# madmann91/bvh

Measured on AMD Instinct MI355X. Metric: Mrays/s closest-hit (1M-tri scene), higher is better.
Workload: dtype f32; 1 GPU; soup_1m: 1,000,000-triangle random soup (M3), worst-case incoherent; robust traversal, DefaultBuilder with thread pool (mini-trees) Quality::High built on the GPU (the reference's default configuration is thread pool + High); rays reordered for coherence inside the timed pass (library default for this tree size); tris=1000000, nodes=1866439, ray_batches=4, parallelism=single GPU, launched_by=single process

## Files before the change

bvh_amd/__init__.py:

```python
from .api import (BinnedSahBuilder, MiniTreeBuilder, SplitHeuristic, Bvh, Config, DefaultBuilder, Quality, RayFlags, SweepSahBuilder, ThreadPool, prepare_trace,
                  HITD, HITF, INVALID, NODED, NODEF, NODE2D, NODE2F, closest_points, hits_to_numpy, intersect, precompute_tris, sphere_bounds,
                  tri_bounds, gather, radius_count, radius_search, offsets_from_counts, ray_hit_count, ray_hits, ray_hits_nearest, RAY_NEAREST_MAX_K, knn, KNN_MAX_K, overlap_count, overlap_search, self_overlaps, instance_prepare, intersect_instanced, std_sort_ids, radix_sort_pairs, reinsertion_stats, last_optimize_profile, pinhole_rays, shade_eyelight)
from ._lib import BvhAmdError
```

bvh_amd/_lib.py:

```python
from __future__ import annotations

import ctypes as C
import os

HERE = os.path.dirname(os.path.abspath(__file__))
LIB_PATH = os.environ.get("BVH_AMD_LIB") or os.path.join(HERE, "lib", "libbvh_amd.so")

_lib = None


class BvhAmdError(RuntimeError):
    pass


class BuildConfig(C.Structure):
    _fields_ = [("quality", C.c_int), ("min_leaf_size", C.c_size_t), ("max_leaf_size", C.c_size_t),
                ("parallel_threshold", C.c_size_t)]


class Counters(C.Structure):
    _fields_ = [("node_pairs", C.c_ulonglong), ("prim_tests", C.c_ulonglong), ("leaves", C.c_ulonglong)]


class MiniTreeConfig(C.Structure):
# ... 58 lines not shown
    "bvh_thread_pool_create": (_P, [_Z]),
    "bvh_thread_pool_destroy": (None, [_P]),
    "bvh_amd_gather": (_I, [_P, _P, _Z, _Z, _P, _P]),
    "bvh_amd_pinhole_rays3f": (_I, [_P, _P, _P, _Z, _Z, _P, _P]),
    "bvh_amd_pinhole_rays3d": (_I, [_P, _P, _P, _Z, _Z, _P, _P]),
    "bvh_amd_shade_eyelight3f": (_I, [_P, _P, _P, _Z, _P, _P]),
    "bvh_amd_shade_eyelight3d": (_I, [_P, _P, _P, _Z, _P, _P]),
    "bvh_amd_device_alloc": (_P, [_Z]),
    "bvh_amd_device_free": (None, [_P]),
    "bvh_amd_copy_to_device": (_I, [_P, _P, _Z]),
    "bvh_amd_copy_to_host": (_I, [_P, _P, _Z]),
    "bvh_amd_synchronize": (_I, [_P]),
    "bvh_amd_std_sort_ids3f": (_I, [_P, _Z, _P, _P]),
    "bvh_amd_std_sort_ids3d": (_I, [_P, _Z, _P, _P]),
    "bvh_amd_radix_sort_pairs_u32": (_I, [_P, _P, _Z, _I, _P]),
    "bvh_amd_offsets_from_counts": (_I, [_P, _Z, _P, _P]),
}
_SIGS_T = {
    "bvh{S}_build": (_P, [_P, _P, _P, _Z, _P]),
    "bvh{S}_build_device": (_P, [_P, _P, _Z, _P, _I, _P]),
    "bvh{S}_build_sah": (_P, [_P, _P, _P, _Z, _P, _P]),
    "bvh{S}_build_device_sah": (_P, [_P, _P, _Z, _P, _I, _P, _P]),
    "bvh{S}_build_device_binned": (_P, [_P, _P, _Z, _P, _P, _Z, _P]),
    "bvh{S}_build_minitree_device": (_P, [_P, _P, _Z, _P, _P]),
    "bvh{S}_from_nodes": (_P, [_P, _Z, _P, _Z]),
    "bvh{S}_extract": (_P, [_P, _Z]),
    "bvh{S}_destroy": (None, [_P]),
    "bvh{S}_optimize": (None, [_P, _P]),
    "bvh{S}_optimize_config": (_I, [_P, _P]),
    "bvh{S}_refit": (None, [_P]),
# ... 136 lines not shown
```

bvh_amd/api.py:

```python
from __future__ import annotations

import ctypes as C
import enum
from dataclasses import dataclass, field

import numpy as np

from . import _lib

INVALID = 0xFFFFFFFF
HITF = np.dtype([("prim", "<u4"), ("t", "<f4"), ("u", "<f4"), ("v", "<f4")])
HITD = np.dtype([("prim", "<u4"), ("pad", "<u4"), ("t", "<f8"), ("u", "<f8"), ("v", "<f8")])
NODEF = np.dtype([("bounds", "<f4", (6,)), ("index", "<u4")])
NODED = np.dtype([("bounds", "<f8", (6,)), ("index", "<u8")])
NODE2F = np.dtype([("bounds", "<f4", (4,)), ("index", "<u4")])
NODE2D = np.dtype([("bounds", "<f8", (4,)), ("index", "<u8")])
_NODE_DTYPES = {"3f": NODEF, "3d": NODED, "2f": NODE2F, "2d": NODE2D}


class Quality(enum.IntEnum):
    Low = 0
    Medium = 1
    High = 2

# ... 758 lines not shown
def std_sort_ids(keys):
    torch = _torch()
    k = _dev(keys).reshape(-1)
    s = _suffix(k.dtype)
    out = torch.empty(k.shape[0], dtype=torch.int32, device=k.device)
    _lib.check(getattr(_lib.load(), f"bvh_amd_std_sort_ids{s}")(k.data_ptr(), k.shape[0], out.data_ptr(), _stream()), "std_sort_ids")
    return out


def radix_sort_pairs(keys_u32, vals_u32, bits=32):
    torch = _torch()
    k = _dev(keys_u32).to(torch.int32).clone()
    v = _dev(vals_u32).to(torch.int32).clone()
    _lib.check(_lib.load().bvh_amd_radix_sort_pairs_u32(k.data_ptr(), v.data_ptr(), k.shape[0], bits, _stream()), "radix_sort_pairs")
    return k, v
```

bvh_amd/csrc/capi.hip:

```cpp
#include "common.h"

#include <cstring>
#include <memory>
#include <type_traits>

namespace bvh_amd {

template <typename T> int reinsertion_optimize_device(HostNode<T>* d_nodes, size_t node_count, hipStream_t stream, int dim);
template <typename T>
int reinsertion_optimize_config_device(HostNode<T>* d_nodes, size_t node_count, hipStream_t stream, int dim, double batch_size_ratio, size_t iterations);
void reinsertion_stats(unsigned out[2]);
void last_optimize_profile(bvh_amd_optimize_profile* out);
template <typename T>
int build_minitree_explicit(BvhImpl<T>& out, const T* d_bboxes, const T* d_centers, size_t n, const bvh_build_config& cfg, bool prune, T ratio,
                            bool optimize, uint32_t log2_grid, hipStream_t stream);
template <typename T>
int extract_device(BvhImpl<T>& out, const HostNode<T>* d_nodes, size_t node_count, const uint32_t* d_ids, size_t root_id, hipStream_t stream);
template <typename T> int refit_device(HostNode<T>* d_nodes, size_t node_count, hipStream_t stream);
template <typename T> int reachable_node_count(const HostNode<T>* d_nodes, size_t node_count, hipStream_t stream, size_t* out);
template <typename T> int relayout_on_device(BvhImpl<T>& b, const HostNode<T>* d_nodes, hipStream_t stream);

namespace {
thread_local std::string g_error;
}
// ... 805 lines not shown
int bvh_amd_std_sort_ids3f(const float* d_keys, size_t n, uint32_t* d_ids_out, void* stream) {
    return std_sort_ids<float>(d_ids_out, d_keys, static_cast<uint32_t>(n), 1, 0, 1, static_cast<hipStream_t>(stream));
}
int bvh_amd_std_sort_ids3d(const double* d_keys, size_t n, uint32_t* d_ids_out, void* stream) {
    return std_sort_ids<double>(d_ids_out, d_keys, static_cast<uint32_t>(n), 1, 0, 1, static_cast<hipStream_t>(stream));
}
int bvh_amd_radix_sort_pairs_u32(uint32_t* d_keys, uint32_t* d_vals, size_t n, int bits, void* stream) {
    DeviceTemps<uint32_t> tmp;
    auto& [kt, vt] = tmp;
    BVH_HIP_TRY(hipMalloc(&kt, std::max<size_t>(n, 1) * 4), BVH_AMD_ERR_HIP);
    hipError_t e = hipMalloc(&vt, std::max<size_t>(n, 1) * 4);
    return e == hipSuccess ? radix_sort_pairs<uint32_t>(d_keys, d_vals, kt, vt, static_cast<uint32_t>(n), 1, bits, static_cast<hipStream_t>(stream))
                           : fail(BVH_AMD_ERR_HIP, hipGetErrorString(e));
}

int bvh_amd_pinhole_rays3f(const float eye[3], const float dir[3], const float up[3], size_t w, size_t h, bvh_ray3f* d_rays, void* stream) {
    return launch_pinhole_rays<float>(eye, dir, up, w, h, reinterpret_cast<float*>(d_rays), static_cast<hipStream_t>(stream));
}
int bvh_amd_pinhole_rays3d(const double eye[3], const double dir[3], const double up[3], size_t w, size_t h, bvh_ray3d* d_rays, void* stream) {
    return launch_pinhole_rays<double>(eye, dir, up, w, h, reinterpret_cast<double*>(d_rays), static_cast<hipStream_t>(stream));
}
int bvh_amd_shade_eyelight3f(const float* d_tris12, const bvh_ray3f* d_rays, const bvh_hit3f* d_hits, size_t n, uint8_t* d_rgb, void* stream) {
    return launch_shade_eyelight<float>(d_tris12, reinterpret_cast<const float*>(d_rays), d_hits, n, d_rgb, static_cast<hipStream_t>(stream));
}
int bvh_amd_shade_eyelight3d(const double* d_tris12, const bvh_ray3d* d_rays, const bvh_hit3d* d_hits, size_t n, uint8_t* d_rgb, void* stream) {
    return launch_shade_eyelight<double>(d_tris12, reinterpret_cast<const double*>(d_rays), d_hits, n, d_rgb, static_cast<hipStream_t>(stream));
}

int bvh_amd_gather(const void* d_in, const uint32_t* d_perm, size_t n, size_t stride, void* d_out, void* stream) {
    return launch_gather(d_in, d_perm, n, stride, d_out, static_cast<hipStream_t>(stream));
// ... 4 lines not shown
```

bvh_amd/csrc/common.h:

```cpp
#pragma once

#include <hip/hip_runtime.h>

#include <cstddef>
#include <cstdint>
#include <cstring>
#include <string>
#include <atomic>
#include <mutex>
#include <vector>

#include "../../include/bvh_amd.h"

namespace bvh_amd {

constexpr unsigned kCountBits = 4;
constexpr uint32_t kCountMask = 15u;
constexpr int kWave = 64;

template <typename T> struct IndexOf;
template <> struct IndexOf<float>  { using Type = uint32_t; };
template <> struct IndexOf<double> { using Type = uint64_t; };

template <typename T>
// ... 216 lines not shown
template <typename T> int launch_sphere_bounds(const T* d_sph4, size_t n, T* d_bb, T* d_cc, hipStream_t s);
int launch_gather(const void* d_in, const uint32_t* d_perm, size_t n, size_t stride, void* d_out, hipStream_t s);
template <typename T> int launch_circle_bounds(const T* d_circles3, size_t n, T* d_bb4, T* d_cc2, hipStream_t s);
template <typename T> int launch_widen_inputs(const T* d_bb4, const T* d_cc2, size_t n, T* d_bb6, T* d_cc3, hipStream_t s);

template <typename T> int launch_pinhole_rays(const T eye[3], const T dir[3], const T up[3], size_t width, size_t height, T* d_rays, hipStream_t s);
template <typename T>
int launch_shade_eyelight(const T* d_tris12, const T* d_rays, const typename HitOf<T>::Type* d_hits, size_t n, uint8_t* d_rgb, hipStream_t s);

template <typename K>
int radix_sort_pairs(K* keys, uint32_t* vals, K* keys_tmp, uint32_t* vals_tmp, uint32_t n, uint32_t batch, int bits, hipStream_t stream,
                     uint32_t* hist_buf = nullptr, bool iota_vals = false, bool keys_wanted = true, uint32_t** vals_result = nullptr,
                     bool first_hist_done = false);
constexpr int kRadixTileU32 = 8192;
size_t radix_sort_hist_words(uint32_t n, uint32_t batch);
template <typename T>
int std_sort_ids(uint32_t* d_ids, const T* d_keys, uint32_t n, uint32_t batch, uint32_t astride, uint32_t istride, hipStream_t stream);

int exclusive_scan_u32(const uint32_t* in, uint32_t* out, uint32_t n, uint32_t* total_host, hipStream_t stream);

template <typename T>
int build_on_device(BvhImpl<T>& out, const T* d_bboxes, const T* d_centers, size_t n, const bvh_build_config& cfg,
                    bvh_amd_builder builder, hipStream_t stream);

enum { LEAF_TRIANGLE = 0, LEAF_SPHERE = 1 };

enum { REFIT_BOXES3 = 0, REFIT_BOXES2 = 1, REFIT_TRIS = 2 };
template <typename T>
int refit_prims_device(HostNode<T>* d_nodes, PairNode<T>* d_pairs, size_t node_count, int src_kind, const T* d_src, size_t n_src,
                       const uint32_t* d_prim_ids, size_t prim_count, hipStream_t stream);
// ... 5 lines not shown
```

bvh_amd/csrc/query_order.h:

```cpp
#pragma once

#include <algorithm>
#include <string>

namespace bvh_amd {

namespace {

enum QueryKind : int { kQueryPoints = 0, kQueryBoxes = 1, kQueryRays = 2 };

template <typename T>
__global__ void __launch_bounds__(1024) closest_keys_kernel(const T* queries, uint32_t n, T lx, T ly, T lz, T sx, T sy, T sz, uint32_t cells,
                                                            uint32_t* keys, uint32_t* hist, uint32_t tiles) {
    __shared__ uint32_t h[256];
    if (threadIdx.x < 256) h[threadIdx.x] = 0;
    __syncthreads();
    const uint32_t base = blockIdx.x * uint32_t(kRadixTileU32);
#pragma unroll
    for (int s0 = 0; s0 < kRadixTileU32 / 1024; ++s0) {
        const uint32_t i = base + uint32_t(s0) * 1024u + threadIdx.x;
        if (i < n) {
            T q[4];
            load_prim4(queries + 4ull * i, q);
            const T r[8] = { q[0], q[1], q[2], T(0), T(0), T(0), T(0), q[3] };
// ... 45 lines not shown
            load_ray(rays + 8ull * i, r);
            const int hilbert_bits = 31 - __clz(cells);
            const uint32_t key = ray_key<T>(r, lx, ly, lz, sx, sy, sz, cells, hilbert_bits, 0, T(0));
            keys[i] = key;
            atomicAdd(&h[key & 0xFFu], 1u);
        }
    }
    __syncthreads();
    if (threadIdx.x < 256) hist[size_t{threadIdx.x} * tiles + blockIdx.x] = h[threadIdx.x];
}

template <typename T, int Kind = kQueryPoints>
int query_order(const BvhImpl<T>& b, const T* d_queries, size_t n, int cell_bits, const char* who, hipStream_t stream, void** sort_mem,
                ScratchTag* sort_tag, const uint32_t** order_out) {
    const uint32_t n32 = static_cast<uint32_t>(n);
    const size_t words = 4 * n + radix_sort_hist_words(n32, 1);
    const hipError_t e = scratch_alloc(sort_mem, words * sizeof(uint32_t), sort_tag);
    if (e != hipSuccess) { *sort_mem = nullptr; return fail(BVH_AMD_ERR_HIP, std::string(who) + ": no scratch for the query sort: " + hipGetErrorString(e)); }
    uint32_t *keys = static_cast<uint32_t*>(*sort_mem), *vals = keys + n, *kt = vals + n, *vt = kt + n, *hist = vt + n;
    const uint32_t cells = 1u << cell_bits;
    T lo[3], sc[3];
    if (const int rc0 = b.wait_refit()) return rc0;
    for (int k = 0; k < 3; ++k) {
        const T ext = b.root_bounds[2 * k + 1] - b.root_bounds[2 * k];
        lo[k] = b.root_bounds[2 * k];
        sc[k] = ext > T(0) ? T(cells) / ext : T(0);
    }
    const uint32_t tiles = (n32 + kRadixTileU32 - 1) / kRadixTileU32;
    if constexpr (Kind == kQueryRays)
        hipLaunchKernelGGL(ray_query_keys_kernel<T>, dim3(tiles), dim3(1024), 0, stream, d_queries, n32, lo[0], lo[1], lo[2], sc[0], sc[1], sc[2], cells,
                           keys, hist, tiles);
    else if constexpr (Kind == kQueryBoxes)
        hipLaunchKernelGGL(box_keys_kernel<T>, dim3(tiles), dim3(1024), 0, stream, d_queries, n32, lo[0], lo[1], lo[2], sc[0], sc[1], sc[2], cells,
                           keys, hist, tiles);
    else
        hipLaunchKernelGGL(closest_keys_kernel<T>, dim3(tiles), dim3(1024), 0, stream, d_queries, n32, lo[0], lo[1], lo[2], sc[0], sc[1], sc[2], cells,
                           keys, hist, tiles);
    BVH_HIP_TRY(hipGetLastError(), BVH_AMD_ERR_HIP);
    uint32_t* order = nullptr;
    const int rc = radix_sort_pairs<uint32_t>(keys, vals, kt, vt, n32, 1, 3 * cell_bits + 3, stream, hist, true, false, &order,
                                              true);
    if (rc) return rc;
    *order_out = order;
    return BVH_AMD_OK;
}

}

}
```

bvh_amd/csrc/sort_emul.hip:

```cpp

#include "build_common.h"

namespace bvh_amd {

using namespace bld;

namespace {

template <typename K> struct RadixShape {
    static constexpr int kTile = sizeof(K) == 2 || sizeof(K) == 4 ? 8192 : 4096;
    static constexpr int kThreads = kTile / 16;
    static constexpr int kWaves = kThreads / 64;
};
constexpr int kRadixMinTile = 4096;

template <typename K>
__global__ void __launch_bounds__(RadixShape<K>::kThreads) k_radix_hist(const K* keys, uint32_t n, uint32_t blocks_per_array, int shift,
                                                                       uint32_t* hist) {
    constexpr int kTile = RadixShape<K>::kTile, kThreads = RadixShape<K>::kThreads;
    __shared__ uint32_t h[256];
    const uint32_t arr = blockIdx.x / blocks_per_array, blk = blockIdx.x % blocks_per_array;
    if (threadIdx.x < 256) h[threadIdx.x] = 0;
    __syncthreads();
    const size_t base = size_t{arr} * n;
// ... 694 lines not shown
        if (!(p == 0 && first_hist_done)) hipLaunchKernelGGL(k_radix_hist<K>, dim3(batch * bpa), dim3(kThreads), 0, stream, kin, n, bpa, shift, hist);
        if (256 * bpa > 16384) {
            for (uint32_t a = 0; a < batch; ++a) {
                int rc = scan_u32_async(hist + size_t{a} * 256 * bpa, hist + size_t{a} * 256 * bpa, 256 * bpa, nullptr, stream);
                if (rc) return rc;
            }
        } else hipLaunchKernelGGL(k_radix_scan, dim3(batch), dim3(1024), 0, stream, hist, 256 * bpa);
        hipLaunchKernelGGL(k_radix_scatter<K>, dim3(batch * bpa), dim3(kThreads), 0, stream, kin, p == 0 && iota_vals ? nullptr : vin,
                           p == passes - 1 && !keys_wanted ? nullptr : kout, vout, n, bpa, shift, hist);
        std::swap(kin, kout);
        std::swap(vin, vout);
    }
    BVH_HIP_TRY(hipGetLastError(), BVH_AMD_ERR_HIP);
    if (vals_result) *vals_result = vin;
    if (!hist_buf && !own.pooled) BVH_HIP_TRY(hipStreamSynchronize(stream), BVH_AMD_ERR_HIP);
    return BVH_AMD_OK;
}

template <typename T>
int std_sort_ids(uint32_t* d_ids, const T* d_keys, uint32_t n, uint32_t batch, uint32_t astride, uint32_t istride, hipStream_t stream) {
    StreamScope scratch_on(stream);
    if (n == 0 || batch == 0) return BVH_AMD_OK;
    static const bool small_off = BVH_DEV_INT("BVH_AMD_SORT_SMALL", 1) == 0;
    if (n <= kSortSmallMax && !small_off) {
        uint32_t lg = 0;
        while ((uint64_t{2} << lg) <= n) ++lg;
        hipLaunchKernelGGL(k_std_sort_small<T>, dim3(batch), dim3(kSortSmallThreads), 0, stream, d_ids, d_keys, n, astride, istride, 2 * lg);
        BVH_HIP_TRY(hipGetLastError(), BVH_AMD_ERR_HIP);
        return BVH_AMD_OK;
    }
// ... 95 lines not shown
```

bvh_amd/csrc/traverse.hip:

```cpp

#include "common.h"
#include "trace_device.h"
#include "ray_key.h"

#include <algorithm>
#include <cstdlib>
#include <mutex>
#include <thread>
#include <type_traits>
#include <vector>

namespace bvh_amd {

namespace {

thread_local const char* g_last_kernel = "";
thread_local bool g_last_reordered = false;
thread_local int g_last_query_launches = 0;
thread_local int g_last_plan[4] = {0, 0, 0, 0};

struct KernelTimer {
    static constexpr size_t kRing = 256;
    bool on = false;
    size_t count = 0;
// ... 63 lines not shown
#pragma unroll
    for (int s0 = 0; s0 < kRadixTileU32 / 1024; ++s0) {
        const uint32_t i = base + uint32_t(s0) * 1024u + threadIdx.x;
        if (i < n) {
            T r[8];
            load_ray_nt(rays + 8ull * i, r);
            const uint32_t key = ray_key<T>(r, lx, ly, lz, sx, sy, sz, cells, hilbert_bits, class_bits, class_scale, tail_frac);
            keys[i] = key;
            atomicAdd(&h[key & 0xFFu], 1u);
        }
    }
    __syncthreads();
    if (threadIdx.x < 256) hist[size_t{threadIdx.x} * tiles + blockIdx.x] = h[threadIdx.x];
}

__global__ void __launch_bounds__(64) ticket_ranges_kernel(const uint32_t* hist, uint32_t tiles, uint32_t digits_per_prefix, uint32_t n, uint32_t parts,
                                                           unsigned long long part_size, uint32_t* starts, unsigned long long* work) {
    const uint32_t p = threadIdx.x;
    uint32_t begin = n, end = n;
    if (p < parts) {
        begin = hist[size_t{p} * digits_per_prefix * tiles];
        if (p + 1 < parts) end = hist[size_t{p + 1} * digits_per_prefix * tiles];
    }
    const uint32_t even = n / parts, len = end - begin;
    const bool balanced = p >= parts || (begin <= end && end <= n && 4ull * len >= 3ull * even && 4ull * len <= 5ull * even);
    const bool keep = __ballot(!balanced) == 0;
    if (p <= parts) starts[p] = keep ? begin : static_cast<uint32_t>(min(static_cast<unsigned long long>(n), p * part_size));
    if (p < parts) work[p * kTicketStride] = 0;
}

__global__ void __launch_bounds__(256) ray_entry_keys_kernel(const float* rays, uint32_t n, const PairNode<float>* pairs, uint32_t root_index, int depth,
                                                             uint32_t* keys) {
    const uint32_t i = blockIdx.x * 256 + threadIdx.x;
    if (i >= n) return;
    float r[8];
    load_ray(rays + 8ull * i, r);
    const float inv[3] = { 1.0f / r[3], 1.0f / r[4], 1.0f / r[5] };
// ... 368 lines not shown
        if (leaf_kind != LEAF_SPHERE) return release(fail(BVH_AMD_ERR_ARG, "intersect_rays: a 2D BVH traces circles (Sphere<T, 2>) only"));
        if (const int rc0 = zero_tickets()) return release(rc0);
        int rc2 = dispatch<T, LEAF_SPHERE, 2>(b, args, flags, d_counters != nullptr, stream);
        if (rc2 == BVH_AMD_OK && (flags & BVH_AMD_RAY_ORIGINAL_IDS)) rc2 = to_original_ids<T>(b, d_hits, n, stream);
        return release(rc2);
    }
    const bool reorder = (flags & BVH_AMD_RAY_SORTED) ? n > 4096
                       : (flags & BVH_AMD_RAY_UNSORTED) ? false
                       : plan ? plan->reorder && n > 4096
                       : n >= (size_t{1} << 20) && beyond_l2 && b.expected_visits.load() >= kReorderMinVisits;
    g_last_reordered = reorder && n < (size_t{1} << 31);
    args.stream_hints = t_exp.stream_hints >= 0 ? static_cast<uint32_t>(t_exp.stream_hints) : g_last_reordered ? 1u : 0u;
    args.parts = t_parts > 0 ? std::min(t_parts, 256) : parts_env > 0 ? std::min(parts_env, 256) : n < 65536 ? 1 : g_last_reordered ? 8 : 32;
    args.part_size = ((n + args.parts - 1) / args.parts + 63) / 64 * 64;
    constexpr size_t kRangeWords = 64;
    if (g_last_reordered) {
        const uint32_t n32 = static_cast<uint32_t>(n);
        const size_t words = 4 * n + radix_sort_hist_words(n32, 1) + kRangeWords;
        hipError_t e = scratch_alloc(&sort_mem, words * sizeof(uint32_t), &sort_tag);
        if (e != hipSuccess) {
            sort_mem = nullptr;
            (void)hipGetLastError();
            if (flags & BVH_AMD_RAY_SORTED) return release(fail(BVH_AMD_ERR_HIP, std::string("intersect_rays: no scratch for BVH_AMD_RAY_SORTED: ") + hipGetErrorString(e)));
            g_last_reordered = false;
        }
    }
    if (!g_last_reordered) {
        if (const int rc0 = zero_tickets()) return release(rc0);
    } else {
        const uint32_t n32 = static_cast<uint32_t>(n);
        uint32_t *keys = static_cast<uint32_t*>(sort_mem), *vals = keys + n, *kt = vals + n, *vt = kt + n, *hist = vt + n;
        T lo[3], sc[3];
        if (const int rc0 = b.wait_refit()) return release(rc0);
        for (int k = 0; k < 3; ++k) {
            const T ext = b.root_bounds[2 * k + 1] - b.root_bounds[2 * k];
            lo[k] = b.root_bounds[2 * k];
            sc[k] = ext > T(0) ? T(64) / ext : T(0);
        }
        static const int entry_depth = std::min(29, BVH_DEV_INT("BVH_AMD_RAY_KEY_DEPTH", 0));
        int key_bits = 21;
        bool entry_keys = false, first_hist_done = false;
        if constexpr (std::is_same_v<T, float>) entry_keys = entry_depth > 0 && b.dim == 3;
        if constexpr (std::is_same_v<T, float>) {
            if (entry_keys) {
                hipLaunchKernelGGL(ray_entry_keys_kernel, dim3((n32 + 255) / 256), dim3(256), 0, stream, d_rays, n32, args.pairs, args.root_index, entry_depth, keys);
                key_bits = entry_depth + 3;
            }
        }
        if (!entry_keys) {
            static const int cell_bits_env = std::max(1, std::min(8, BVH_DEV_INT("BVH_AMD_RAY_KEY_BITS", 7)));
            const int cell_bits = t_exp.key_bits > 0 ? std::min(8, t_exp.key_bits) : cell_bits_env;
            const T rescale = static_cast<T>(1u << cell_bits) / T(64);
            const int class_bits = cell_bits < 3 ? 0 : t_exp.key_class_bits >= 0 ? std::min(3, t_exp.key_class_bits) : (plan && plan->classes) ? 1 : kKeyClassBits;
            g_last_classes = class_bits > 0;
            const T class_scale = static_cast<T>(t_exp.key_class_scale > 0 ? t_exp.key_class_scale : kKeyClassScalePercent) / T(100);
            const bool tail = class_bits == 1 && cell_bits >= 2 && (t_exp.key_tail >= 0 ? t_exp.key_tail > 0 : kKeyTail > 0);
            const T tail_frac = tail ? static_cast<T>(t_exp.key_tail_permille >= 0 ? t_exp.key_tail_permille : kKeyTailPermille) / T(1000) : T(-1);
            const uint32_t tiles = (n32 + kRadixTileU32 - 1) / kRadixTileU32;
            hipLaunchKernelGGL(ray_keys_kernel<T>, dim3(tiles), dim3(1024), 0, stream, d_rays, n32, lo[0], lo[1], lo[2], sc[0] * rescale, sc[1] * rescale,
                               sc[2] * rescale, keys, 1u << cell_bits, t_exp.key_curve == 0 ? 0 : cell_bits,
                               class_bits, class_scale, tail_frac, hist, tiles);
            first_hist_done = true;
            key_bits = 3 * cell_bits + 3;
        }
        uint32_t* order = nullptr;
        int rc = radix_sort_pairs<uint32_t>(keys, vals, kt, vt, n32, 1, key_bits, stream, hist, true, false, &order, first_hist_done);
        if (rc) return release(rc);
        args.order = order;
        const int top_digit_bits = key_bits - 8 * ((key_bits + 7) / 8 - 1);
        const bool align = args.parts == 8 && !args.one_shot && top_digit_bits >= 3 && (t_exp.range_align >= 0 ? t_exp.range_align > 0 : kRangeAlign > 0);
        if (align) {
            uint32_t* starts = hist + radix_sort_hist_words(n32, 1);
            const uint32_t tiles = (n32 + kRadixTileU32 - 1) / kRadixTileU32;
            hipLaunchKernelGGL(ticket_ranges_kernel, dim3(1), dim3(64), 0, stream, hist, tiles, 1u << (top_digit_bits - 3), n32, args.parts, args.part_size, starts, work);
            if (const hipError_t e = hipGetLastError(); e != hipSuccess) return release(fail(BVH_AMD_ERR_HIP, std::string("intersect_rays: ticket_ranges_kernel: ") + hipGetErrorString(e)));
            args.range_starts = starts;
        } else if (const int rc0 = zero_tickets()) return release(rc0);
#if defined(BVH_AMD_DEVELOPER)
        if (getenv("BVH_AMD_CHECK_ORDER")) {
            uint32_t* d_bad = nullptr;
            if (hipMalloc(&d_bad, 8 * sizeof(uint32_t)) == hipSuccess) {
                for (int round = 0; round < 2; ++round) {
                    (void)hipMemsetAsync(d_bad, 0, 8 * sizeof(uint32_t), stream);
                    hipLaunchKernelGGL(k_check_order, dim3((n32 + 255) / 256), dim3(256), 0, stream, order, n32, d_bad);
                    uint32_t bad[8] = {};
                    (void)hipMemcpyAsync(bad, d_bad, sizeof(bad), hipMemcpyDeviceToHost, stream);
                    (void)hipStreamSynchronize(stream);
                    if (bad[0]) {
                        std::vector<uint32_t> host(n32);
// ... 172 lines not shown
        if (rc == BVH_AMD_OK) ps.recorded = true;
        else ps.pending = false;
    }
    return rc;
}

template <typename T>
int prepare_trace(const BvhImpl<T>& b, size_t n_rays_hint, hipStream_t stream) {
    if (b.node_count == 0) return BVH_AMD_OK;
    if (b.pair_count && !b.d_pairs) return fail(BVH_AMD_ERR_ARG, "prepare_trace: BVH has no device nodes");
    if (const int rc = tree_depth<T>(b, stream)) return rc;
    if (n_rays_hint >= (size_t{1} << 20) && n_rays_hint < (size_t{1} << 31) && scratch_pool_enabled()) {
        StreamScope scope(stream);
        void* mem = nullptr;
        ScratchTag tag;
        const size_t words = 4 * n_rays_hint + radix_sort_hist_words(static_cast<uint32_t>(n_rays_hint), 1);
        if (scratch_alloc(&mem, words * sizeof(uint32_t), &tag) == hipSuccess) scratch_free(mem, tag);
        else (void)hipGetLastError();
    }
    return BVH_AMD_OK;
}
template int prepare_trace<float>(const BvhImpl<float>&, size_t, hipStream_t);
template int prepare_trace<double>(const BvhImpl<double>&, size_t, hipStream_t);

template int launch_traverse<float>(const BvhImpl<float>&, int, const float*, const float*, size_t, unsigned,
                                    bvh_hit3f*, bvh_amd_counters*, hipStream_t);
template int launch_traverse<double>(const BvhImpl<double>&, int, const double*, const double*, size_t, unsigned,
                                     bvh_hit3d*, bvh_amd_counters*, hipStream_t);

}
```

include/bvh_amd.h:

```cpp
#ifndef BVH_AMD_H
#define BVH_AMD_H

#include <stddef.h>
#include <stdint.h>
#include <stdio.h>
#include <stdbool.h>

#ifdef __cplusplus
extern "C" {
#endif

#define BVH_AMD_API __attribute__((visibility("default")))

#define BVH_ROOT_INDEX 0
#define BVH_INVALID_PRIM_ID SIZE_MAX

struct bvh3f;
struct bvh3d;
struct bvh_node3f;
struct bvh_node3d;
struct bvh2f;
struct bvh2d;
struct bvh_node2f;
struct bvh_node2d;
// ... 319 lines not shown
BVH_AMD_API int bvh3d_instance_prepare(const struct bvh_amd_geometry3d* geoms, size_t n_geoms, const double* d_obj2world12, const uint32_t* d_geometry,
    size_t n_instances, double* d_world2obj12, double* d_bboxes, double* d_centers, void* stream);
BVH_AMD_API int bvh3f_intersect_rays_instanced(const struct bvh3f* top, const struct bvh_amd_geometry3f* geoms, size_t n_geoms,
    const float* d_world2obj12, const uint32_t* d_geometry, size_t n_instances, const struct bvh_ray3f* d_rays, size_t n_rays, unsigned flags,
    struct bvh_hit3f* d_hits, uint32_t* d_hit_instances, struct bvh_amd_counters* d_counters, void* stream);
BVH_AMD_API int bvh3d_intersect_rays_instanced(const struct bvh3d* top, const struct bvh_amd_geometry3d* geoms, size_t n_geoms,
    const double* d_world2obj12, const uint32_t* d_geometry, size_t n_instances, const struct bvh_ray3d* d_rays, size_t n_rays, unsigned flags,
    struct bvh_hit3d* d_hits, uint32_t* d_hit_instances, struct bvh_amd_counters* d_counters, void* stream);

BVH_AMD_API int bvh3f_prepare_trace(const struct bvh3f*, size_t n_rays_hint, void* stream);
BVH_AMD_API int bvh3d_prepare_trace(const struct bvh3d*, size_t n_rays_hint, void* stream);

BVH_AMD_API int bvh_amd_std_sort_ids3f(const float* d_keys, size_t n, uint32_t* d_ids_out, void* stream);
BVH_AMD_API int bvh_amd_std_sort_ids3d(const double* d_keys, size_t n, uint32_t* d_ids_out, void* stream);
BVH_AMD_API int bvh_amd_radix_sort_pairs_u32(uint32_t* d_keys, uint32_t* d_vals, size_t n, int bits, void* stream);

BVH_AMD_API const char* bvh_amd_last_kernel_name(void);
BVH_AMD_API int bvh_amd_last_launch_reordered(void);
BVH_AMD_API int bvh_amd_last_query_launches(void);
BVH_AMD_API void bvh_amd_kernel_timing(int on);
BVH_AMD_API int bvh_amd_kernel_times(float* ms_out, size_t capacity, size_t* count_out);
BVH_AMD_API int bvh_amd_reorder_times(float* ms_out, size_t capacity, size_t* count_out);
BVH_AMD_API void bvh_amd_tuning(int refill_threshold, int leaf_threshold, int coop_fetch, int ticket_ranges);
BVH_AMD_API int bvh_amd_experiment(const char* name, int value);
BVH_AMD_API int bvh_amd_wave_times(unsigned long long* out, size_t capacity_waves, size_t* n_waves);
BVH_AMD_API void bvh_amd_last_launch_plan(int out[4]);
BVH_AMD_API void bvh_amd_last_plan_search(float ns_per_ray[5], int measurements[5], unsigned* dropped_mask);
BVH_AMD_API void bvh_amd_reinsertion_stats(unsigned out[2]);
struct bvh_amd_optimize_profile { unsigned iterations, replayed; unsigned long long replacements; float heap_ms; };
BVH_AMD_API void bvh_amd_last_optimize_profile(struct bvh_amd_optimize_profile* out);
// ... 133 lines not shown
```

Measured before the change: 2555 Mrays/s.

## Add order-only radix sort with shrinking key carries for ray reordering

Adds a dedicated radix sort that produces only the permutation. The first pass generates indices itself (16-bit local in shared memory), and later passes carry only the remaining key bits as 8- or 16-bit values instead of full 32-bit keys and values. The ray and query reordering paths use it, and the ticket range kernel now reads per-digit totals and scans them in-wave instead of reading the global histogram prefix layout. This is meant to cut the memory traffic of the in-pass ray sort, at the cost of more specialised kernels and a changed scratch layout.

```diff
diff --git a/bvh_amd/__init__.py b/bvh_amd/__init__.py
--- a/bvh_amd/__init__.py
+++ b/bvh_amd/__init__.py
@@ -1,4 +1,4 @@
 from .api import (BinnedSahBuilder, MiniTreeBuilder, SplitHeuristic, Bvh, Config, DefaultBuilder, Quality, RayFlags, SweepSahBuilder, ThreadPool, prepare_trace,
                   HITD, HITF, INVALID, NODED, NODEF, NODE2D, NODE2F, closest_points, hits_to_numpy, intersect, precompute_tris, sphere_bounds,
-                  tri_bounds, gather, radius_count, radius_search, offsets_from_counts, ray_hit_count, ray_hits, ray_hits_nearest, RAY_NEAREST_MAX_K, knn, KNN_MAX_K, overlap_count, overlap_search, self_overlaps, instance_prepare, intersect_instanced, std_sort_ids, radix_sort_pairs, reinsertion_stats, last_optimize_profile, pinhole_rays, shade_eyelight)
+                  tri_bounds, gather, radius_count, radius_search, offsets_from_counts, ray_hit_count, ray_hits, ray_hits_nearest, RAY_NEAREST_MAX_K, knn, KNN_MAX_K, overlap_count, overlap_search, self_overlaps, instance_prepare, intersect_instanced, std_sort_ids, radix_sort_pairs, radix_order, reinsertion_stats, last_optimize_profile, pinhole_rays, shade_eyelight)
 from ._lib import BvhAmdError
diff --git a/bvh_amd/_lib.py b/bvh_amd/_lib.py
--- a/bvh_amd/_lib.py
+++ b/bvh_amd/_lib.py
@@ -96,6 +96,7 @@
     "bvh_amd_std_sort_ids3f": (_I, [_P, _Z, _P, _P]),
     "bvh_amd_std_sort_ids3d": (_I, [_P, _Z, _P, _P]),
     "bvh_amd_radix_sort_pairs_u32": (_I, [_P, _P, _Z, _I, _P]),
+    "bvh_amd_radix_order_u32": (_I, [_P, _Z, _I, _P, _P]),
     "bvh_amd_offsets_from_counts": (_I, [_P, _Z, _P, _P]),
 }
 _SIGS_T = {
diff --git a/bvh_amd/api.py b/bvh_amd/api.py
--- a/bvh_amd/api.py
+++ b/bvh_amd/api.py
@@ -796,3 +796,11 @@
     v = _dev(vals_u32).to(torch.int32).clone()
     _lib.check(_lib.load().bvh_amd_radix_sort_pairs_u32(k.data_ptr(), v.data_ptr(), k.shape[0], bits, _stream()), "radix_sort_pairs")
     return k, v
+
+
+def radix_order(keys_u32, bits=32):
+    torch = _torch()
+    k = _dev(keys_u32).to(torch.int32).contiguous()
+    out = torch.empty(k.shape[0], dtype=torch.int32, device=k.device)
+    _lib.check(_lib.load().bvh_amd_radix_order_u32(k.data_ptr(), k.shape[0], bits, out.data_ptr(), _stream()), "radix_order")
+    return out
diff --git a/bvh_amd/csrc/capi.hip b/bvh_amd/csrc/capi.hip
--- a/bvh_amd/csrc/capi.hip
+++ b/bvh_amd/csrc/capi.hip
@@ -843,6 +843,11 @@
                            : fail(BVH_AMD_ERR_HIP, hipGetErrorString(e));
 }
 
+int bvh_amd_radix_order_u32(const uint32_t* d_keys, size_t n, int bits, uint32_t* d_order_out, void* stream) {
+    if (n >= (size_t{1} << 31)) return fail(BVH_AMD_ERR_ARG, "bvh_amd_radix_order_u32: fewer than 2^31 keys");
+    return radix_order_of_keys(d_keys, static_cast<uint32_t>(n), bits, d_order_out, static_cast<hipStream_t>(stream));
+}
+
 int bvh_amd_pinhole_rays3f(const float eye[3], const float dir[3], const float up[3], size_t w, size_t h, bvh_ray3f* d_rays, void* stream) {
     return launch_pinhole_rays<float>(eye, dir, up, w, h, reinterpret_cast<float*>(d_rays), static_cast<hipStream_t>(stream));
 }
diff --git a/bvh_amd/csrc/common.h b/bvh_amd/csrc/common.h
--- a/bvh_amd/csrc/common.h
+++ b/bvh_amd/csrc/common.h
@@ -254,6 +254,10 @@
                      bool first_hist_done = false);
 constexpr int kRadixTileU32 = 8192;
 size_t radix_sort_hist_words(uint32_t n, uint32_t batch);
+struct RadixOrderLayout { size_t carry, vals0, vals1, hist, words; };
+RadixOrderLayout radix_order_layout(uint32_t n, int bits);
+int radix_sort_order(uint32_t* scratch, uint32_t n, int bits, hipStream_t stream, bool first_hist_done, uint32_t** order);
+int radix_order_of_keys(const uint32_t* d_keys, uint32_t n, int bits, uint32_t* d_order, hipStream_t stream);
 template <typename T>
 int std_sort_ids(uint32_t* d_ids, const T* d_keys, uint32_t n, uint32_t batch, uint32_t astride, uint32_t istride, hipStream_t stream);
 
diff --git a/bvh_amd/csrc/query_order.h b/bvh_amd/csrc/query_order.h
--- a/bvh_amd/csrc/query_order.h
+++ b/bvh_amd/csrc/query_order.h
@@ -83,10 +83,11 @@
 int query_order(const BvhImpl<T>& b, const T* d_queries, size_t n, int cell_bits, const char* who, hipStream_t stream, void** sort_mem,
                 ScratchTag* sort_tag, const uint32_t** order_out) {
     const uint32_t n32 = static_cast<uint32_t>(n);
-    const size_t words = 4 * n + radix_sort_hist_words(n32, 1);
-    const hipError_t e = scratch_alloc(sort_mem, words * sizeof(uint32_t), sort_tag);
+    const int key_bits = 3 * cell_bits + 3;
+    const RadixOrderLayout layout = radix_order_layout(n32, key_bits);
+    const hipError_t e = scratch_alloc(sort_mem, layout.words * sizeof(uint32_t), sort_tag);
     if (e != hipSuccess) { *sort_mem = nullptr; return fail(BVH_AMD_ERR_HIP, std::string(who) + ": no scratch for the query sort: " + hipGetErrorString(e)); }
-    uint32_t *keys = static_cast<uint32_t*>(*sort_mem), *vals = keys + n, *kt = vals + n, *vt = kt + n, *hist = vt + n;
+    uint32_t *keys = static_cast<uint32_t*>(*sort_mem), *hist = keys + layout.hist;
     const uint32_t cells = 1u << cell_bits;
     T lo[3], sc[3];
     if (const int rc0 = b.wait_refit()) return rc0;
@@ -107,8 +108,7 @@
                            keys, hist, tiles);
     BVH_HIP_TRY(hipGetLastError(), BVH_AMD_ERR_HIP);
     uint32_t* order = nullptr;
-    const int rc = radix_sort_pairs<uint32_t>(keys, vals, kt, vt, n32, 1, 3 * cell_bits + 3, stream, hist, true, false, &order,
-                                              true);
+    const int rc = radix_sort_order(keys, n32, key_bits, stream, true, &order);
     if (rc) return rc;
     *order_out = order;
     return BVH_AMD_OK;
diff --git a/bvh_amd/csrc/sort_emul.hip b/bvh_amd/csrc/sort_emul.hip
--- a/bvh_amd/csrc/sort_emul.hip
+++ b/bvh_amd/csrc/sort_emul.hip
@@ -732,6 +732,258 @@
     BVH_HIP_TRY(hipGetLastError(), BVH_AMD_ERR_HIP);
     if (vals_result) *vals_result = vin;
     if (!hist_buf && !own.pooled) BVH_HIP_TRY(hipStreamSynchronize(stream), BVH_AMD_ERR_HIP);
+    return BVH_AMD_OK;
+}
+
+namespace {
+
+constexpr int kOrderTile = kRadixTileU32, kOrderThreads = kOrderTile / 16, kOrderWaves = kOrderThreads / 64;
+
+__global__ void __launch_bounds__(1024) k_order_copy_keys(const uint32_t* in, uint32_t n, uint32_t* keys, uint32_t* hist, uint32_t tiles) {
+    __shared__ uint32_t h[256];
+    if (threadIdx.x < 256) h[threadIdx.x] = 0;
+    __syncthreads();
+    const uint32_t base = blockIdx.x * uint32_t(kOrderTile);
+    for (int s0 = 0; s0 < kOrderTile / 1024; ++s0) {
+        const uint32_t i = base + uint32_t(s0) * 1024u + threadIdx.x;
+        if (i < n) {
+            const uint32_t key = in[i];
+            keys[i] = key;
+            atomicAdd(&h[key & 0xFFu], 1u);
+        }
+    }
+    __syncthreads();
+    if (threadIdx.x < 256) hist[size_t{threadIdx.x} * tiles + blockIdx.x] = h[threadIdx.x];
+}
+
+template <typename K>
+__global__ void __launch_bounds__(kOrderThreads) k_order_hist(const K* keys, uint32_t n, uint32_t tiles, uint32_t* hist) {
+    constexpr uint32_t kPer = 4 / sizeof(K);
+    __shared__ uint32_t h[256];
+    if (threadIdx.x < 256) h[threadIdx.x] = 0;
+    __syncthreads();
+    const uint32_t b = blockIdx.x * uint32_t(kOrderTile), e = min(n, b + uint32_t(kOrderTile));
+    const uint32_t* w = reinterpret_cast<const uint32_t*>(keys + b);
+    const uint32_t words = (e - b + kPer - 1) / kPer;
+    for (uint32_t j = threadIdx.x; j < words; j += uint32_t(kOrderThreads)) {
+        const uint32_t v = w[j];
+#pragma unroll
+        for (uint32_t k = 0; k < kPer; ++k)
+            if (b + j * kPer + k < e) atomicAdd(&h[(v >> (8 * sizeof(K) * k)) & 0xFFu], 1u);
+    }
+    __syncthreads();
+    if (threadIdx.x < 256) hist[size_t{threadIdx.x} * tiles + blockIdx.x] = h[threadIdx.x];
+}
+
+__global__ void __launch_bounds__(256) k_order_scan(uint32_t* hist, uint32_t tiles) {
+    constexpr int kItems = 8;
+    __shared__ uint32_t wsum[4];
+    uint32_t* h = hist + size_t{blockIdx.x} * tiles;
+    const int lane = threadIdx.x & 63, wave = threadIdx.x >> 6;
+    uint32_t run = 0;
+    for (uint32_t c0 = 0; c0 < tiles; c0 += 256 * kItems) {
+        const uint32_t i0 = c0 + threadIdx.x * kItems;
+        uint32_t v[kItems], s = 0;
+#pragma unroll
+        for (int k = 0; k < kItems; ++k) { v[k] = i0 + k < tiles ? h[i0 + k] : 0u; s += v[k]; }
+        uint32_t inc = s;
+#pragma unroll
+        for (int d = 1; d < 64; d <<= 1) {
+            const uint32_t o = __shfl_up(inc, d);
+            if (lane >= d) inc += o;
+        }
+        if (lane == 63) wsum[wave] = inc;
+        __syncthreads();
+        uint32_t at = run + inc - s, total = 0;
+        for (int w = 0; w < 4; ++w) { if (w < wave) at += wsum[w]; total += wsum[w]; }
+#pragma unroll
+        for (int k = 0; k < kItems; ++k) { if (i0 + k < tiles) h[i0 + k] = at; at += v[k]; }
+        run += total;
+        __syncthreads();
+    }
+    if (threadIdx.x == 0) hist[size_t{256} * tiles + blockIdx.x] = run;
+}
+
+template <typename KI, typename KO, bool KeysOut, bool Iota>
+__global__ void __launch_bounds__(kOrderThreads) k_order_scatter(const KI* keys, const uint32_t* vals, KO* keys_out, uint32_t* vals_out, uint32_t n,
+                                                                 uint32_t tiles, const uint32_t* hist) {
+    constexpr int kTile = kOrderTile, kThreads = kOrderThreads, kWaves = kOrderWaves, kSteps = 16;
+    constexpr bool kWholeKey = KeysOut && sizeof(KO) == 4;
+    using V = std::conditional_t<Iota, uint16_t, uint32_t>;
+    __shared__ uint32_t cursor[kWaves][128];
+    __shared__ V sval[kTile];
+    __shared__ KO skey[KeysOut ? kTile : 1];
+    __shared__ uint8_t sdig[kWholeKey ? 1 : kTile];
+    static_assert(sizeof(V) * kTile >= 2 * 256 * sizeof(uint32_t) && sizeof(cursor) >= 256 * sizeof(uint32_t));
+    uint32_t* const part = reinterpret_cast<uint32_t*>(sval);
+    uint32_t* const dpart = part + 256;
+    uint32_t* const delta = &cursor[0][0];
+    const uint32_t blk = blockIdx.x;
+    const int lane = threadIdx.x & 63, wave = threadIdx.x >> 6;
+    for (int i = threadIdx.x; i < kWaves * 128; i += kThreads) (&cursor[0][0])[i] = 0;
+    __syncthreads();
+    const uint32_t b = blk * uint32_t(kTile), e = min(n, b + uint32_t(kTile));
+    const uint32_t first = b + wave * uint32_t(kSteps * 64) + lane;
+    uint32_t* mine = cursor[wave];
+    KI key[kSteps]; V val[kSteps];
+#pragma unroll
+    for (int s = 0; s < kSteps; ++s) {
+        const uint32_t i = first + s * 64;
+        key[s] = 0; val[s] = 0;
+        if (i < e) {
+            key[s] = keys[i];
+            if constexpr (Iota) val[s] = static_cast<V>(i - b); else val[s] = vals[i];
+            const uint32_t d = key[s] & 0xFF;
+            atomicAdd(&mine[d >> 1], 1u << (16 * (d & 1)));
+        }
+    }
+    __syncthreads();
+    uint32_t total = 0, dtotal = 0;
+    if (threadIdx.x < 256) {
+#pragma unroll
+        for (int w = 0; w < kWaves; ++w) total += (cursor[w][threadIdx.x >> 1] >> (16 * (threadIdx.x & 1))) & 0xFFFFu;
+        part[threadIdx.x] = total;
+        dtotal = hist[size_t{256} * tiles + threadIdx.x];
+        dpart[threadIdx.x] = dtotal;
+    }
+    __syncthreads();
+    for (int off = 1; off < 256; off <<= 1) {
+        uint32_t v = 0, dv = 0;
+        if (threadIdx.x < 256 && int(threadIdx.x) >= off) { v = part[threadIdx.x - off]; dv = dpart[threadIdx.x - off]; }
+        __syncthreads();
+        if (threadIdx.x < 256) { part[threadIdx.x] += v; dpart[threadIdx.x] += dv; }
+        __syncthreads();
+    }
+    uint32_t my_delta = 0;
+    if (threadIdx.x < 256) {
+        const uint32_t start = part[threadIdx.x] - total;
+        my_delta = (dpart[threadIdx.x] - dtotal) + hist[size_t{threadIdx.x} * tiles + blk] - start;
+        part[threadIdx.x] = start;
+    }
+    __syncthreads();
+    if (threadIdx.x < 128) {
+        uint32_t r0 = part[2 * threadIdx.x], r1 = part[2 * threadIdx.x + 1];
+#pragma unroll
+        for (int w = 0; w < kWaves; ++w) {
+            const uint32_t c = cursor[w][threadIdx.x];
+            cursor[w][threadIdx.x] = r0 | (r1 << 16);
+            r0 += c & 0xFFFFu; r1 += c >> 16;
+        }
+    }
+    __syncthreads();
+    const uint64_t below = (uint64_t{1} << lane) - 1;
+#pragma unroll
+    for (int s = 0; s < kSteps; ++s) {
+        const bool in = first + s * 64 < e;
+        const uint32_t d = key[s] & 0xFF;
+        uint64_t same = __ballot(in);
+#pragma unroll
+        for (int bit = 0; bit < 8; ++bit) {
+            const uint64_t bal = __ballot((d >> bit) & 1);
+            same &= ((d >> bit) & 1) ? bal : ~bal;
+        }
+        if (in) {
+            const uint32_t rank = __popcll(same & below);
+            const uint32_t at = (mine[d >> 1] >> (16 * (d & 1))) & 0xFFFFu;
+            __builtin_amdgcn_wave_barrier();
+            if (rank == 0) atomicAdd(&mine[d >> 1], uint32_t(__popcll(same)) << (16 * (d & 1)));
+            if constexpr (kWholeKey) skey[at + rank] = key[s];
+            else {
+                if constexpr (KeysOut) skey[at + rank] = static_cast<KO>(key[s] >> 8);
+                sdig[at + rank] = static_cast<uint8_t>(d);
+            }
+            sval[at + rank] = val[s];
+        }
+        __builtin_amdgcn_wave_barrier();
+    }
+    __syncthreads();
+    if (threadIdx.x < 256) delta[threadIdx.x] = my_delta;
+    __syncthreads();
+    for (uint32_t j = threadIdx.x; j < e - b; j += uint32_t(kThreads)) {
+        if constexpr (kWholeKey) {
+            const KO k = skey[j];
+            const uint32_t at = j + delta[k & 0xFF];
+            keys_out[at] = k >> 8;
+            vals_out[at] = Iota ? b + sval[j] : sval[j];
+        } else {
+            const uint32_t at = j + delta[sdig[j]];
+            if constexpr (KeysOut) keys_out[at] = skey[j];
+            vals_out[at] = Iota ? b + sval[j] : sval[j];
+        }
+    }
+}
+
+inline int order_carry_bytes(int left) { return left <= 0 ? 0 : left <= 8 ? 1 : left <= 16 ? 2 : 4; }
+
+}
+
+RadixOrderLayout radix_order_layout(uint32_t n, int bits) {
+    const int passes = std::max(1, (bits + 7) / 8);
+    const size_t tiles = (size_t{n} + kOrderTile - 1) / kOrderTile;
+    auto pad = [](size_t words) { return (words + 3) / 4 * 4; };
+    RadixOrderLayout l;
+    l.carry = pad(n);
+    l.vals0 = l.carry + pad((size_t{n} * order_carry_bytes(bits - 8) + 3) / 4);
+    l.vals1 = l.vals0 + pad(n);
+    l.hist = l.vals1 + (passes > 1 ? pad(n) : 0);
+    l.words = l.hist + 256 * tiles + 256;
+    return l;
+}
+
+int radix_sort_order(uint32_t* scratch, uint32_t n, int bits, hipStream_t stream, bool first_hist_done, uint32_t** order) {
+    if (bits < 1 || bits > 32) return fail(BVH_AMD_ERR_ARG, "radix_sort_order: 1..32 key bits");
+    const RadixOrderLayout l = radix_order_layout(n, bits);
+    uint32_t* const hist = scratch + l.hist;
+    uint32_t* vbuf[2] = { scratch + l.vals0, scratch + l.vals1 };
+    void* kbuf[2] = { scratch, scratch + l.carry };
+    *order = vbuf[0];
+    if (n == 0) return BVH_AMD_OK;
+    const uint32_t tiles = (n + kOrderTile - 1) / kOrderTile;
+    const int passes = (bits + 7) / 8;
+    int in_bytes = 4;
+    for (int p = 0; p < passes; ++p) {
+        const int out_bytes = order_carry_bytes(bits - 8 * (p + 1));
+        const void* kin = kbuf[p & 1]; void* kout = kbuf[(p + 1) & 1];
+        const uint32_t* vin = p == 0 ? nullptr : vbuf[(p + 1) & 1];
+        uint32_t* vout = vbuf[p & 1];
+        const dim3 grid(tiles), block(kOrderThreads);
+        if (!(p == 0 && first_hist_done)) {
+            if (in_bytes == 4) hipLaunchKernelGGL(k_order_hist<uint32_t>, grid, block, 0, stream, static_cast<const uint32_t*>(kin), n, tiles, hist);
+            else if (in_bytes == 2) hipLaunchKernelGGL(k_order_hist<uint16_t>, grid, block, 0, stream, static_cast<const uint16_t*>(kin), n, tiles, hist);
+            else hipLaunchKernelGGL(k_order_hist<uint8_t>, grid, block, 0, stream, static_cast<const uint8_t*>(kin), n, tiles, hist);
+        }
+        hipLaunchKernelGGL(k_order_scan, dim3(256), dim3(256), 0, stream, hist, tiles);
+#define BVH_ORDER_SCATTER(KI, KO, OUT, IOTA) \
+        hipLaunchKernelGGL((k_order_scatter<KI, KO, OUT, IOTA>), grid, block, 0, stream, static_cast<const KI*>(kin), vin, static_cast<KO*>(kout), vout, n, tiles, hist)
+        if (p == 0 && out_bytes == 4) BVH_ORDER_SCATTER(uint32_t, uint32_t, true, true);
+        else if (p == 0 && out_bytes == 2) BVH_ORDER_SCATTER(uint32_t, uint16_t, true, true);
+        else if (p == 0 && out_bytes == 1) BVH_ORDER_SCATTER(uint32_t, uint8_t, true, true);
+        else if (p == 0) BVH_ORDER_SCATTER(uint32_t, uint8_t, false, true);
+        else if (in_bytes == 4 && out_bytes == 2) BVH_ORDER_SCATTER(uint32_t, uint16_t, true, false);
+        else if (in_bytes == 2 && out_bytes == 1) BVH_ORDER_SCATTER(uint16_t, uint8_t, true, false);
+        else if (in_bytes == 1 && out_bytes == 0) BVH_ORDER_SCATTER(uint8_t, uint8_t, false, false);
+        else return fail(BVH_AMD_ERR_ARG, "radix_sort_order: no kernel for this hand-over of key types");
+#undef BVH_ORDER_SCATTER
+        *order = vout;
+        in_bytes = out_bytes;
+    }
+    BVH_HIP_TRY(hipGetLastError(), BVH_AMD_ERR_HIP);
+    return BVH_AMD_OK;
+}
+
+int radix_order_of_keys(const uint32_t* d_keys, uint32_t n, int bits, uint32_t* d_order, hipStream_t stream) {
+    if (bits < 1 || bits > 32) return fail(BVH_AMD_ERR_ARG, "radix_order_of_keys: 1..32 key bits");
+    if (n == 0) return BVH_AMD_OK;
+    StreamScope scratch_on(stream);
+    const RadixOrderLayout l = radix_order_layout(n, bits);
+    DevBuf<uint32_t> scratch;
+    BVH_HIP_TRY(scratch.alloc(l.words), BVH_AMD_ERR_HIP);
+    const uint32_t tiles = (n + kOrderTile - 1) / kOrderTile;
+    hipLaunchKernelGGL(k_order_copy_keys, dim3(tiles), dim3(1024), 0, stream, d_keys, n, scratch.p, scratch.p + l.hist, tiles);
+    uint32_t* order = nullptr;
+    if (const int rc = radix_sort_order(scratch.p, n, bits, stream, true, &order)) return rc;
+    BVH_HIP_TRY(hipMemcpyAsync(d_order, order, size_t{n} * 4, hipMemcpyDeviceToDevice, stream), BVH_AMD_ERR_HIP);
+    if (!scratch.pooled) BVH_HIP_TRY(hipStreamSynchronize(stream), BVH_AMD_ERR_HIP);
     return BVH_AMD_OK;
 }
 
diff --git a/bvh_amd/csrc/traverse.hip b/bvh_amd/csrc/traverse.hip
--- a/bvh_amd/csrc/traverse.hip
+++ b/bvh_amd/csrc/traverse.hip
@@ -101,13 +101,21 @@
     if (threadIdx.x < 256) hist[size_t{threadIdx.x} * tiles + blockIdx.x] = h[threadIdx.x];
 }
 
-__global__ void __launch_bounds__(64) ticket_ranges_kernel(const uint32_t* hist, uint32_t tiles, uint32_t digits_per_prefix, uint32_t n, uint32_t parts,
+__global__ void __launch_bounds__(64) ticket_ranges_kernel(const uint32_t* totals, uint32_t digits_per_prefix, uint32_t n, uint32_t parts,
                                                            unsigned long long part_size, uint32_t* starts, unsigned long long* work) {
     const uint32_t p = threadIdx.x;
+    uint32_t mine = 0;
+    if (p < parts) for (uint32_t d = p * digits_per_prefix; d < (p + 1) * digits_per_prefix; ++d) mine += totals[d];
+    uint32_t upto = mine;
+#pragma unroll
+    for (int off = 1; off < 64; off <<= 1) {
+        const uint32_t o = __shfl_up(upto, off);
+        if (int(p) >= off) upto += o;
+    }
     uint32_t begin = n, end = n;
     if (p < parts) {
-        begin = hist[size_t{p} * digits_per_prefix * tiles];
-        if (p + 1 < parts) end = hist[size_t{p + 1} * digits_per_prefix * tiles];
+        begin = upto - mine;
+        if (p + 1 < parts) end = upto;
     }
     const uint32_t even = n / parts, len = end - begin;
     const bool balanced = p >= parts || (begin <= end && end <= n && 4ull * len >= 3ull * even && 4ull * len <= 5ull * even);
@@ -506,9 +514,17 @@
     args.parts = t_parts > 0 ? std::min(t_parts, 256) : parts_env > 0 ? std::min(parts_env, 256) : n < 65536 ? 1 : g_last_reordered ? 8 : 32;
     args.part_size = ((n + args.parts - 1) / args.parts + 63) / 64 * 64;
     constexpr size_t kRangeWords = 64;
+    static const int entry_depth = std::min(29, BVH_DEV_INT("BVH_AMD_RAY_KEY_DEPTH", 0));
+    static const int cell_bits_env = std::max(1, std::min(8, BVH_DEV_INT("BVH_AMD_RAY_KEY_BITS", 7)));
+    const int cell_bits = t_exp.key_bits > 0 ? std::min(8, t_exp.key_bits) : cell_bits_env;
+    bool entry_keys = false;
+    if constexpr (std::is_same_v<T, float>) entry_keys = entry_depth > 0 && b.dim == 3;
+    const int key_bits = entry_keys ? entry_depth + 3 : 3 * cell_bits + 3;
+    RadixOrderLayout sort_layout{};
     if (g_last_reordered) {
         const uint32_t n32 = static_cast<uint32_t>(n);
-        const size_t words = 4 * n + radix_sort_hist_words(n32, 1) + kRangeWords;
+        sort_layout = radix_order_layout(n32, key_bits);
+        const size_t words = sort_layout.words + kRangeWords;
         hipError_t e = scratch_alloc(&sort_mem, words * sizeof(uint32_t), &sort_tag);
         if (e != hipSuccess) {
             sort_mem = nullptr;
@@ -521,7 +537,7 @@
         if (const int rc0 = zero_tickets()) return release(rc0);
     } else {
         const uint32_t n32 = static_cast<uint32_t>(n);
-        uint32_t *keys = static_cast<uint32_t*>(sort_mem), *vals = keys + n, *kt = vals + n, *vt = kt + n, *hist = vt + n;
+        uint32_t *keys = static_cast<uint32_t*>(sort_mem), *hist = keys + sort_layout.hist;
         T lo[3], sc[3];
         if (const int rc0 = b.wait_refit()) return release(rc0);
         for (int k = 0; k < 3; ++k) {
@@ -529,19 +545,12 @@
             lo[k] = b.root_bounds[2 * k];
             sc[k] = ext > T(0) ? T(64) / ext : T(0);
         }
-        static const int entry_depth = std::min(29, BVH_DEV_INT("BVH_AMD_RAY_KEY_DEPTH", 0));
-        int key_bits = 21;
-        bool entry_keys = false, first_hist_done = false;
-        if constexpr (std::is_same_v<T, float>) entry_keys = entry_depth > 0 && b.dim == 3;
+        bool first_hist_done = false;
         if constexpr (std::is_same_v<T, float>) {
-            if (entry_keys) {
+            if (entry_keys)
                 hipLaunchKernelGGL(ray_entry_keys_kernel, dim3((n32 + 255) / 256), dim3(256), 0, stream, d_rays, n32, args.pairs, args.root_index, entry_depth, keys);
-                key_bits = entry_depth + 3;
-            }
         }
         if (!entry_keys) {
-            static const int cell_bits_env = std::max(1, std::min(8, BVH_DEV_INT("BVH_AMD_RAY_KEY_BITS", 7)));
-            const int cell_bits = t_exp.key_bits > 0 ? std::min(8, t_exp.key_bits) : cell_bits_env;
             const T rescale = static_cast<T>(1u << cell_bits) / T(64);
             const int class_bits = cell_bits < 3 ? 0 : t_exp.key_class_bits >= 0 ? std::min(3, t_exp.key_class_bits) : (plan && plan->classes) ? 1 : kKeyClassBits;
             g_last_classes = class_bits > 0;
@@ -553,18 +562,17 @@
                                sc[2] * rescale, keys, 1u << cell_bits, t_exp.key_curve == 0 ? 0 : cell_bits,
                                class_bits, class_scale, tail_frac, hist, tiles);
             first_hist_done = true;
-            key_bits = 3 * cell_bits + 3;
         }
         uint32_t* order = nullptr;
-        int rc = radix_sort_pairs<uint32_t>(keys, vals, kt, vt, n32, 1, key_bits, stream, hist, true, false, &order, first_hist_done);
+        int rc = radix_sort_order(keys, n32, key_bits, stream, first_hist_done, &order);
         if (rc) return release(rc);
         args.order = order;
         const int top_digit_bits = key_bits - 8 * ((key_bits + 7) / 8 - 1);
         const bool align = args.parts == 8 && !args.one_shot && top_digit_bits >= 3 && (t_exp.range_align >= 0 ? t_exp.range_align > 0 : kRangeAlign > 0);
         if (align) {
-            uint32_t* starts = hist + radix_sort_hist_words(n32, 1);
+            uint32_t* starts = keys + sort_layout.words;
             const uint32_t tiles = (n32 + kRadixTileU32 - 1) / kRadixTileU32;
-            hipLaunchKernelGGL(ticket_ranges_kernel, dim3(1), dim3(64), 0, stream, hist, tiles, 1u << (top_digit_bits - 3), n32, args.parts, args.part_size, starts, work);
+            hipLaunchKernelGGL(ticket_ranges_kernel, dim3(1), dim3(64), 0, stream, hist + size_t{256} * tiles, 1u << (top_digit_bits - 3), n32, args.parts, args.part_size, starts, work);
             if (const hipError_t e = hipGetLastError(); e != hipSuccess) return release(fail(BVH_AMD_ERR_HIP, std::string("intersect_rays: ticket_ranges_kernel: ") + hipGetErrorString(e)));
             args.range_starts = starts;
         } else if (const int rc0 = zero_tickets()) return release(rc0);
@@ -767,7 +775,7 @@
         StreamScope scope(stream);
         void* mem = nullptr;
         ScratchTag tag;
-        const size_t words = 4 * n_rays_hint + radix_sort_hist_words(static_cast<uint32_t>(n_rays_hint), 1);
+        const size_t words = radix_order_layout(static_cast<uint32_t>(n_rays_hint), 24).words + 64;
         if (scratch_alloc(&mem, words * sizeof(uint32_t), &tag) == hipSuccess) scratch_free(mem, tag);
         else (void)hipGetLastError();
     }
diff --git a/include/bvh_amd.h b/include/bvh_amd.h
--- a/include/bvh_amd.h
+++ b/include/bvh_amd.h
@@ -357,6 +357,7 @@
 BVH_AMD_API int bvh_amd_std_sort_ids3f(const float* d_keys, size_t n, uint32_t* d_ids_out, void* stream);
 BVH_AMD_API int bvh_amd_std_sort_ids3d(const double* d_keys, size_t n, uint32_t* d_ids_out, void* stream);
 BVH_AMD_API int bvh_amd_radix_sort_pairs_u32(uint32_t* d_keys, uint32_t* d_vals, size_t n, int bits, void* stream);
+BVH_AMD_API int bvh_amd_radix_order_u32(const uint32_t* d_keys, size_t n, int bits, uint32_t* d_order_out, void* stream);
 
 BVH_AMD_API const char* bvh_amd_last_kernel_name(void);
 BVH_AMD_API int bvh_amd_last_launch_reordered(void);
```

New measurement: 2605 Mrays/s (median of 6 runs). +1.9%, better.
